# ashvardanian/StringZilla

Measured on AMD Instinct MI355X. Metric: DP cell-updates/s (GCUPS) on 1M-pair Levenshtein batch, higher is better.
Workload: dtype u32 bit-vectors (u64 results)

## Files before the change

### stringzilla_amd/csrc/hip/lev_myers.hip

```cpp
#include "myers_core.hpp"

#define SZS_PAIR_RULE_FN __host__ __device__ static inline
#include "pair_rule.h"
#define SZS_CORNER_CUT_FN __host__ __device__ static inline
#include "corner_cut.h"

#include <cstdlib>

namespace szs_hip {

#ifndef SZS_MYERS_PACK_QUERIES
#define SZS_MYERS_PACK_QUERIES 1
#endif
#ifndef SZS_MYERS_PAIR_RULES
#define SZS_MYERS_PAIR_RULES 1
#endif

#ifndef SZS_MYERS_CUT_CORNERS
#define SZS_MYERS_CUT_CORNERS 1
#endif

#ifndef SZS_MYERS_SHORT_TEXT_DWORDS
#define SZS_MYERS_SHORT_TEXT_DWORDS 2
#endif


__device__ __forceinline__ u32 bits_in_word(u32 from, u32 to, int w) {
    u32 const low = from > 32u * w ? from : 32u * w, high = to < 32u * w + 32u ? to : 32u * w + 32u;
    if (low >= high) return 0u;
    return (high - low == 32u ? ~0u : (1u << (high - low)) - 1u) << (low - 32u * w);
}

template <int words_, int text_dwords_, bool runes_, bool paired_ = false>
__device__ __forceinline__ void myers_workgroup(u32 *peq, u32 *keys, szs_string_ref_t const query,
                                                szs_string_ref_t const *__restrict__ candidates, u32 candidates_count,
                                                u32 candidate_block, u64 *__restrict__ results, u64 results_row_stride,
                                                int symmetric, szs_ref_guard_t const &guard, u32 alphabet = 0,
                                                u32 *claimed_rows = nullptr, u32 blocks_here = 1, szs_string_ref_t const second = {}) {
    static_assert(!paired_ || !runes_, "query pairs are a byte-kernel shape");
    constexpr int rows = runes_ ? rune_slots_k : byte_rows_k;
    using layout = peq_layout<words_, rows>;
    if (guard.enabled && (!ref_is_current(guard, 0, query) || (paired_ && !ref_is_current(guard, 0, second)))) {
        if (threadIdx.x == 0) *guard.stale = guard.sequence;
        return;
    }
    u32 const first_length = query.length, second_length = paired_ ? second.length : 0u;
    u32 const query_length = paired_ ? first_length + second_length : first_length;
    u32 const used_rows = paired_ ? query_length + 2u : query_length;
    u32 const pad = 32u * words_ - used_rows;
    u32 const second_row = pad + first_length + 2u;

    if constexpr (paired_) {
        u32 const s0_dword = (second_row - 2u) >> 5, s0_mask = 1u << ((second_row - 2u) & 31u);
        for (int i = threadIdx.x; i < layout::total_dwords; i += 256)
            peq[i] = (u32)(i / (rows * layout::chunk_words) * layout::chunk_words + i % layout::chunk_words) == s0_dword ? s0_mask : 0u;
    }
    else
        for (int i = threadIdx.x; i < layout::total_dwords; i += 256) peq[i] = 0;
    if constexpr (runes_) {
        if (alphabet) {
            for (u32 i = threadIdx.x; i <= alphabet; i += 256) keys[i] = 0;
            if (threadIdx.x == 0) *claimed_rows = 0;
        }
        else
            for (int i = threadIdx.x; i < rune_slots_k; i += 256) keys[i] = rune_slot_empty_k;
    }
    __syncthreads();
    if (runes_ && alphabet) {
        u32 const *pattern = reinterpret_cast<u32 const *>(query.address);
        for (u32 i = threadIdx.x; i < query_length; i += 256) {
            u32 const id = pattern[i];
            if (atomicCAS(&keys[id], 0u, ~0u) == 0u) keys[id] = atomicAdd(claimed_rows, 1u) + 1;
        }
        __syncthreads();
        for (u32 i = threadIdx.x; i < query_length; i += 256) {
            u32 const position = pad + i;
            atomicOr(&peq[layout::dword_index((int)keys[pattern[i]], (int)(position >> 5))], 1u << (position & 31));
        }
    }
    else if constexpr (runes_) {
        u32 const *pattern = reinterpret_cast<u32 const *>(query.address);
        for (u32 i = threadIdx.x; i < query_length; i += 256) {
            u32 const rune = pattern[i];
            u32 slot = rune_slot_hash(rune);
            for (;;) {
                u32 const previous = atomicCAS(&keys[slot], rune_slot_empty_k, rune);
                if (previous == rune_slot_empty_k || previous == rune) break;
                slot = (slot + 1) & (rune_slots_k - 1);
            }
            u32 const position = pad + i;
            atomicOr(&peq[layout::dword_index((int)slot, (int)(position >> 5))], 1u << (position & 31));
        }
    }
    else {
        u8 const *pattern = reinterpret_cast<u8 const *>(query.address);
        for (u32 i = threadIdx.x; i < first_length; i += 256) {
            u32 const position = pad + i;
            atomicOr(&peq[layout::dword_index(pattern[i], (int)(position >> 5))], 1u << (position & 31));
        }
        if constexpr (paired_) {
            u8 const *above = reinterpret_cast<u8 const *>(second.address);
            for (u32 i = threadIdx.x; i < second_length; i += 256) {
                u32 const position = second_row + i;
                atomicOr(&peq[layout::dword_index(above[i], (int)(position >> 5))], 1u << (position & 31));
            }
        }
    }
    __syncthreads();
    pattern_pair_t<words_> boundary;
    if constexpr (paired_) {
#pragma unroll
        for (int w = 0; w < words_; ++w) {
            boundary.separators[w] = bits_in_word(second_row - 2u, second_row, w);
            boundary.lower[w] = bits_in_word(second_row - 2u, second_row - 1u, w);
        }
    }

#pragma unroll 1
    for (u32 block_step = 0; block_step < blocks_here; ++block_step) {
    u32 const candidate_slot = (candidate_block - block_step) * SZS_CANDIDATES_PER_WORKGROUP + threadIdx.x;
    bool live = candidate_slot < candidates_count;
    szs_string_ref_t candidate = {0, 0, 0};
    if (live) candidate = candidates[candidate_slot];
    if (live && guard.enabled && !ref_is_current(guard, 1, candidate)) {
        *guard.stale = guard.sequence;
        live = false;
    }
    if ((symmetric & SZS_LAYOUT_SYMMETRIC) && candidate.index > query.index) live = false;
    u32 const text_length = live ? candidate.length : 0;
    u32 const longest_in_wave = wave_max_u32(text_length);
    u32 const shortest_in_wave = ~wave_max_u32(live ? ~text_length : 0u);

    u32 vp[words_], vn[words_];
#pragma unroll
    for (int w = 0; w < words_; ++w) {
        vp[w] = bits_in_word(pad, 32u * words_, w) & ~(paired_ ? boundary.separators[w] : 0u);
        vn[w] = 0;
    }

    auto take_words = [&](u32 symbol, auto first_word, auto last_word) {
        constexpr int first = decltype(first_word)::value, last = decltype(last_word)::value;
        u32 eq[words_];
        load_match_masks<words_, rows, first, last>(peq, !runes_ ? symbol : alphabet ? keys[symbol] : find_rune_slot(keys, symbol), eq);
        if constexpr (paired_) myers_column<words_, pattern_pair_t<words_>, true, true, first, last>(vp, vn, eq, boundary);
        else myers_column<words_, single_pattern_t, true, true, first, last>(vp, vn, eq);
    };
    constexpr std::integral_constant<int, 0> word_zero{};
    constexpr std::integral_constant<int, words_> word_end{};
    auto take = [&](u32 symbol) { take_words(symbol, word_zero, word_end); };

    u32 column = 0;
    if constexpr (runes_) {
        u32 const *const runes = reinterpret_cast<u32 const *>(candidate.address);
        auto quad_at = [&](u32 index) -> uint4 {
            return index < text_length ? *reinterpret_cast<uint4 const *>(runes + index) : make_uint4(0, 0, 0, 0);
        };
        if (4 <= shortest_in_wave && longest_in_wave) {
            uint4 ahead = quad_at(0);
            for (; column + 4 <= shortest_in_wave; column += 4) {
                uint4 const now = ahead;
                ahead = quad_at(column + 4);
                take(now.x), take(now.y), take(now.z), take(now.w);
            }
        }
#pragma unroll 1
        for (; column < longest_in_wave; ++column)
            if (column < text_length) take(runes[column]);
    }
    else {
        u64 const safe_address = text_length ? candidate.address : first_length || !paired_ ? query.address : second.address;
        text_stream_t text(safe_address, text_length);
        if (!text_length) text.valid_dwords = query_length ? 1 : 0;
        u32 raw_low = text.raw(0);
        u32 dword = 0;
        constexpr u32 columns_per_iteration = 4 * text_dwords_;
#ifndef SZS_MYERS_CLAMPED_READS
#define SZS_MYERS_CLAMPED_READS(TEXT_DWORDS) ((TEXT_DWORDS) == 1)
#endif
        constexpr bool clamped_reads = SZS_MYERS_CLAMPED_READS(text_dwords_);
        constexpr bool phases = SZS_MYERS_CUT_CORNERS && !runes_ && words_ >= (int)SZS_CORNER_CUT_WORDS_LEAST && text_dwords_ > 1;
        constexpr std::integral_constant<int, phases ? 1 : 0> word_one{};
        constexpr std::integral_constant<int, phases ? words_ - 1 : words_> word_top{};
        u32 head_until = 0, late_from = SZS_CORNER_CUT_NEVER;
        if constexpr (phases)
            szs_corner_cut(first_length, second_length, paired_, words_, (u32)__builtin_amdgcn_readfirstlane((int)shortest_in_wave),
                           (u32)__builtin_amdgcn_readfirstlane((int)longest_in_wave), &head_until, &late_from);
        if (columns_per_iteration <= shortest_in_wave && longest_in_wave && query_length) {
            u32 ahead[text_dwords_];
#pragma unroll
            for (int d = 0; d < text_dwords_; ++d) ahead[d] = clamped_reads ? text.raw_clamped(1 + d) : text.raw(1 + d);
            auto batch = [&](auto first_word, auto last_word) {
                u32 symbols[text_dwords_];
                symbols[0] = text.splice(raw_low, ahead[0]);
#pragma unroll
                for (int d = 1; d < text_dwords_; ++d) symbols[d] = text.splice(ahead[d - 1], ahead[d]);
                raw_low = ahead[text_dwords_ - 1];
#pragma unroll
                for (int d = 0; d < text_dwords_; ++d)
                    ahead[d] = clamped_reads ? text.raw_clamped(dword + text_dwords_ + 1 + d)
                                             : text.raw(dword + text_dwords_ + 1 + d);
#pragma unroll
                for (int step = 0; step < 4 * text_dwords_; ++step)
                    take_words((symbols[step / 4] >> (8 * (step % 4))) & 0xFFu, first_word, last_word);
                column += columns_per_iteration, dword += text_dwords_;
            };
            if constexpr (phases) {
                u32 const shortest = (u32)__builtin_amdgcn_readfirstlane((int)shortest_in_wave);
                u32 const head_end = head_until < shortest ? head_until : shortest;
                while (column + columns_per_iteration <= head_end) batch(word_zero, word_top);
            }
            while (column + columns_per_iteration <= shortest_in_wave && (!phases || column < late_from)) batch(word_zero, word_end);
            if constexpr (phases)
                while (column + columns_per_iteration <= shortest_in_wave) batch(word_one, word_end);
        }
#ifndef SZS_MYERS_MID_LOOP
#define SZS_MYERS_MID_LOOP 0
#endif
        if constexpr (SZS_MYERS_MID_LOOP && text_dwords_ > 1) {
            if (column + 4 <= shortest_in_wave && longest_in_wave && query_length) {
                u32 ahead_one = text.raw(dword + 1);
#pragma unroll 1
                for (; column + 4 <= shortest_in_wave; column += 4, ++dword) {
                    u32 const symbols = text.splice(raw_low, ahead_one);
                    raw_low = ahead_one;
                    ahead_one = text.raw(dword + 2);
#pragma unroll
                    for (int step = 0; step < 4; ++step) take((symbols >> (8 * step)) & 0xFFu);
                }
            }
        }
        if (column < longest_in_wave) {
            u32 next = text.raw(dword + 1);
#pragma unroll 1
            for (; column < longest_in_wave; column += 4, ++dword) {
                u32 const after = text.raw(dword + 2);
                u32 const symbols = text.splice(raw_low, next);
                raw_low = next, next = after;
                if (phases && column >= late_from) {
#pragma unroll
                    for (int step = 0; step < 4; ++step)
                        if (column + step < text_length) take_words((symbols >> (8 * step)) & 0xFFu, word_one, word_end);
                    continue;
                }
#pragma unroll
                for (int step = 0; step < 4; ++step)
                    if (column + step < text_length) take((symbols >> (8 * step)) & 0xFFu);
            }
        }
    }

    if (live && paired_) {
        u32 first = text_length, above = text_length;
#pragma unroll
        for (int w = 0; w < words_; ++w) {
            u32 const mine = bits_in_word(pad, pad + first_length, w), theirs = bits_in_word(second_row, 32u * words_, w);
            first += (u32)__builtin_popcount(vp[w] & mine) - (u32)__builtin_popcount(vn[w] & mine);
            above += (u32)__builtin_popcount(vp[w] & theirs) - (u32)__builtin_popcount(vn[w] & theirs);
        }
        bool const transposed = (symmetric & SZS_LAYOUT_TRANSPOSED) != 0;
        u64 const one = transposed ? candidate.index : query.index, two = transposed ? candidate.index : second.index;
        u64 const one_column = transposed ? query.index : candidate.index, two_column = transposed ? second.index : candidate.index;
        results[one * results_row_stride + one_column] = first;
        results[two * results_row_stride + two_column] = above;
    }
    else if (live) {
        u32 distance = text_length;
#pragma unroll
        for (int w = 0; w < words_; ++w) distance += (u32)__builtin_popcount(vp[w]) - (u32)__builtin_popcount(vn[w]);
        bool const transposed = (symmetric & SZS_LAYOUT_TRANSPOSED) != 0;
        u64 const row = transposed ? candidate.index : query.index, column = transposed ? query.index : candidate.index;
        results[row * results_row_stride + column] = distance;
        if ((symmetric & SZS_LAYOUT_SYMMETRIC) && candidate.index != query.index)
            results[column * results_row_stride + row] = distance;
    }
    }
}

#ifndef SZS_WORK_BLOCK_MAJOR
#define SZS_WORK_BLOCK_MAJOR 1
#endif
__device__ __forceinline__ void myers_work_item(u32 candidate_blocks, u32 &query_slot, u32 &candidate_block) {
#if SZS_WORK_BLOCK_MAJOR
    u32 const queries_count = gridDim.x / candidate_blocks;
    query_slot = blockIdx.x % queries_count;
    candidate_block = candidate_blocks - 1 - blockIdx.x / queries_count;
#else
    query_slot = blockIdx.x / candidate_blocks;
    candidate_block = candidate_blocks - 1 - blockIdx.x % candidate_blocks;
#endif
}

#ifndef SZS_MYERS_LONG_WAVES
#define SZS_MYERS_LONG_WAVES 2
#endif
template <int words_>
__global__ __launch_bounds__(256, SZS_MYERS_LONG_WAVES) void levenshtein_myers_long_kernel(szs_string_ref_t const *__restrict__ queries,
                                                                      szs_string_ref_t const *__restrict__ candidates,
                                                                      u32 candidates_count, u32 candidate_blocks,
                                                                      u64 *__restrict__ results, u64 results_row_stride,
                                                                      int symmetric, szs_ref_guard_t guard) {
    __shared__ __attribute__((aligned(16))) u32 peq[peq_layout<words_>::total_dwords];
    u32 query_slot, candidate_block;
    myers_work_item(candidate_blocks, query_slot, candidate_block);
    myers_workgroup<words_, 1, false>(peq, nullptr, queries[query_slot], candidates, candidates_count, candidate_block,
                                      results, results_row_stride, symmetric, guard);
}

__device__ __forceinline__ u64 fused_offset(void const *offsets, u32 wide, u64 index) {
    return wide ? static_cast<u64 const *>(offsets)[index] : (u64) static_cast<u32 const *>(offsets)[index];
}

__device__ __forceinline__ void fused_sort_side(szs_plan_side_t const &side, u32 is_query_side, u32 choose_rule, u32 sequence, u32 *ready,
                                                u32 second_ready, u32 withhold, szs_fused_side_report_t *report, u32 *histogram ,
                                                szs_string_ref_t *staged ) {
    constexpr u32 per_thread = SZS_FUSED_MOST_STRINGS / 256;
    u32 const tid = threadIdx.x, lane = tid & 63u, wave = tid >> 6, count = side.count;
    bool const one_pass = count <= SZS_FUSED_MOST_STRINGS;
    __shared__ u32 wave_bins[4], wave_longest[4], wave_status[4];
    __shared__ unsigned long long wave_symbols[4], wave_bands_systolic[4], wave_bands_chain[4], wave_squares[4];
    __shared__ u32 rule_words[256];

    u64 const began = wall_clock64();
    for (u32 bin = tid; bin < SZS_FUSED_BINS; bin += 256) histogram[bin] = 0;
    u64 from[per_thread], to[per_thread];
#pragma unroll
    for (u32 k = 0; k < per_thread; ++k) {
        u32 const i = tid + k * 256;
        from[k] = to[k] = 0;
        if (one_pass && i < count) from[k] = fused_offset(side.offsets, side.wide, i), to[k] = fused_offset(side.offsets, side.wide, (u64)i + 1);
    }
    __syncthreads();
    u32 bins[per_thread];
    u32 status = 0, longest = 0;
    u64 symbols = 0, bands_systolic = 0, bands_chain = 0, squares = 0;
    auto count_in = [&](u64 first, u64 last) -> u32 {
        if (last < first) return status |= SZS_PLAN_STATUS_DESCENDING, ~0u;
        if (last - first > 0xFFFFFFFFull) return status |= SZS_PLAN_STATUS_OVERFLOW, ~0u;
        u32 const length = (u32)(last - first);
        symbols += length, squares += (u64)length * length, longest = length > longest ? length : longest;
        bands_systolic += length ? (length + SZS_SYSTOLIC_BAND_ROWS - 1) / SZS_SYSTOLIC_BAND_ROWS : 1;
        bands_chain += length ? (length + SZS_MYERS_CHAIN_BAND_ROWS - 1) / SZS_MYERS_CHAIN_BAND_ROWS : 1;
        u32 const bin = length < SZS_FUSED_BINS - 1 ? length : SZS_FUSED_BINS - 1;
        atomicAdd(&histogram[bin], 1u);
        return bin;
    };
    if (one_pass) {
#pragma unroll
        for (u32 k = 0; k < per_thread; ++k) {
            bins[k] = ~0u;
            if (tid + k * 256 < count) bins[k] = count_in(from[k], to[k]);
        }
    }
    else {
#pragma unroll 1
        for (u32 first = 0; first < count; first += 1024) {
            u64 some_from[4], some_to[4];
#pragma unroll
            for (u32 k = 0; k < 4; ++k) {
                u32 const i = first + tid + k * 256;
                some_from[k] = some_to[k] = 0;
                if (i < count) some_from[k] = fused_offset(side.offsets, side.wide, i), some_to[k] = fused_offset(side.offsets, side.wide, (u64)i + 1);
            }
#pragma unroll
            for (u32 k = 0; k < 4; ++k)
                if (first + tid + k * 256 < count) (void)count_in(some_from[k], some_to[k]);
        }
// ... 70 lines not shown
                some_from[k] = some_to[k] = 0;
                if (i < count) some_from[k] = fused_offset(side.offsets, side.wide, i), some_to[k] = fused_offset(side.offsets, side.wide, (u64)i + 1);
            }
#pragma unroll
            for (u32 k = 0; k < 4; ++k) {
                u32 const i = first + tid + k * 256;
                if (i >= count) continue;
                u32 const length = status ? 0u : (u32)(some_to[k] - some_from[k]);
                szs_string_ref_t ref;
                ref.address = status ? side.base : side.base + some_from[k], ref.length = blank ? 0u : length, ref.index = i;
                u32 const position = status ? i : atomicAdd(&histogram[length < SZS_FUSED_BINS - 1 ? length : SZS_FUSED_BINS - 1], 1u);
                side.ascending[position] = ref, side.descending[count - 1 - position] = ref;
            }
        }
    }
    __syncthreads();
    if (tid == 0) report->ticks[3] = (u32)(wall_clock64() - began);
    u32 pairing = 0;
    if (choosing && wave == 0) {
        constexpr u32 strides = 256 / SZS_PAIR_RULE_CANDIDATES;
        u32 key = ~0u;
        if (lane < SZS_PAIR_RULE_CANDIDATES) {
            u32 total = 0;
#pragma unroll
            for (u32 k = 0; k < strides; ++k) total += rule_words[lane + k * SZS_PAIR_RULE_CANDIDATES];
            key = (total << 5) | lane;
        }
#pragma unroll
        for (int offset = 16; offset >= 1; offset >>= 1) {
            u32 const other = (u32)__shfl_xor((int)key, offset, 64);
            key = other < key ? other : key;
        }
        pairing = szs_pair_rule_candidate(key & 31u, pair_seconds);
    }
    if (tid == 0) {
        if (!withhold) {
            if (is_query_side)
                __hip_atomic_store(reinterpret_cast<u64 *>(ready), ((u64)pairing << 32) | sequence, __ATOMIC_RELEASE, __HIP_MEMORY_SCOPE_AGENT);
            else
                __hip_atomic_store(ready, sequence, __ATOMIC_RELEASE, __HIP_MEMORY_SCOPE_AGENT);
            if (second_ready) __hip_atomic_store(ready + 32, sequence, __ATOMIC_RELAXED, __HIP_MEMORY_SCOPE_AGENT);
        }
        report->ticks[4] = (u32)(wall_clock64() - began);
    }
#pragma unroll
    for (int offset = 32; offset >= 1; offset >>= 1) {
        symbols += ((u64)(u32)__shfl_xor((int)(u32)(symbols >> 32), offset, 64) << 32) | (u32)__shfl_xor((int)(u32)symbols, offset, 64);
        squares += ((u64)(u32)__shfl_xor((int)(u32)(squares >> 32), offset, 64) << 32) | (u32)__shfl_xor((int)(u32)squares, offset, 64);
        bands_systolic += ((u64)(u32)__shfl_xor((int)(u32)(bands_systolic >> 32), offset, 64) << 32) | (u32)__shfl_xor((int)(u32)bands_systolic, offset, 64);
        bands_chain += ((u64)(u32)__shfl_xor((int)(u32)(bands_chain >> 32), offset, 64) << 32) | (u32)__shfl_xor((int)(u32)bands_chain, offset, 64);
    }
    if (lane == 0) wave_symbols[wave] = symbols, wave_bands_systolic[wave] = bands_systolic, wave_bands_chain[wave] = bands_chain, wave_squares[wave] = squares;
    if (tid <= SZS_PLAN_RANK_SAMPLES) {
        u32 const rank = (u32)((u64)tid * (count ? count - 1 : 0) / SZS_PLAN_RANK_SAMPLES);
        report->rank_lengths[tid] = status || !count ? 0u : one_pass ? staged[rank].length : side.ascending[rank].length;
    }
    __syncthreads();
    if (tid == 0) {
        report->status = status, report->blank = blank, report->pairing = pairing;
        report->stats.count = count, report->stats.longest = longest;
        report->stats.symbols = wave_symbols[0] + wave_symbols[1] + wave_symbols[2] + wave_symbols[3];
        report->stats.bands_systolic = wave_bands_systolic[0] + wave_bands_systolic[1] + wave_bands_systolic[2] + wave_bands_systolic[3];
        report->stats.bands_chain = wave_bands_chain[0] + wave_bands_chain[1] + wave_bands_chain[2] + wave_bands_chain[3];
        report->squares = wave_squares[0] + wave_squares[1] + wave_squares[2] + wave_squares[3];
        report->sequence = sequence;
    }
}

__device__ __forceinline__ bool fused_prologue(szs_fused_plan_t const &plan, u32 *scratch, u32 &pairing) {
    __shared__ __attribute__((aligned(16))) szs_string_ref_t staged[SZS_FUSED_MOST_STRINGS];
    for (u32 s = 0; s < (plan.symmetric ? 1u : 2u); ++s)
        if (blockIdx.x == s % gridDim.x) {
            fused_sort_side(plan.side[s], s == 0, SZS_MYERS_PAIR_RULES && SZS_MYERS_PACK_QUERIES && s == 0 && !plan.symmetric && plan.blocks_per_group == 1,
                            plan.sequence, plan.ready + 32 * s, plan.symmetric, plan.withhold, plan.report + s, scratch, staged);
            __syncthreads();
        }
    __shared__ u32 unpublished[2], published_high[2];
    if (threadIdx.x < 2) {
        u32 polls = 0;
        u64 word;
        bool published;
        while (!(published = (u32)(word = __hip_atomic_load(reinterpret_cast<u64 const *>(plan.ready + 32 * threadIdx.x), __ATOMIC_RELAXED,
                                                             __HIP_MEMORY_SCOPE_AGENT)) == plan.sequence) &&
               ++polls < plan.poll_budget)
            __builtin_amdgcn_s_sleep(8);
        unpublished[threadIdx.x] = !published, published_high[threadIdx.x] = (u32)(word >> 32);
    }
    __syncthreads();
    pairing = (u32)__builtin_amdgcn_readfirstlane((int)published_high[0]);
    if (unpublished[0] | unpublished[1]) {
        if (threadIdx.x == 0) __hip_atomic_store(plan.gave_up, plan.sequence, __ATOMIC_RELAXED, __HIP_MEMORY_SCOPE_SYSTEM);
        return false;
    }
    return true;
}

#ifndef SZS_MYERS_SHORT_WAVES
#define SZS_MYERS_SHORT_WAVES 1
#endif
constexpr u32 szs_myers_pair_words_k = SZS_PAIR_WORDS_MOST;
template <bool runes_, bool merged_, bool fused_ = false>
__device__ __forceinline__ void myers_short_body(
    szs_string_ref_t const *__restrict__ queries, szs_string_ref_t const *__restrict__ candidates, u32 candidates_count,
    u32 candidate_blocks, u64 *__restrict__ results, u64 results_row_stride, int symmetric, szs_ref_guard_t guard, u32 alphabet,
    u32 blocks_per_group, szs_fused_plan_t const *fused = nullptr) {
    constexpr bool pairs = fused_ && !merged_ && SZS_MYERS_PACK_QUERIES;
    __shared__ __attribute__((aligned(16))) u32 peq[peq_layout<pairs ? szs_myers_pair_words_k : 8, runes_ ? rune_slots_k : byte_rows_k>::total_dwords];
    u32 pairing = 0;
    if constexpr (fused_) {
        static_assert(peq_layout<8, byte_rows_k>::total_dwords >= SZS_FUSED_BINS, "the sort's histogram borrows the masks' LDS");
        if (!fused_prologue(*fused, peq, pairing)) return;
    }
    __shared__ u32 slot_keys[runes_ ? rune_slots_k : 1];
    __shared__ u32 claimed_rows;
    extern __shared__ u32 rows_of_ids[];
    u32 *const keys = runes_ && alphabet ? rows_of_ids : slot_keys;
    u32 query_slot, candidate_group;
    myers_work_item(candidate_blocks, query_slot, candidate_group);
    u32 const all_blocks = (candidates_count + SZS_CANDIDATES_PER_WORKGROUP - 1) / SZS_CANDIDATES_PER_WORKGROUP;
    u32 const first_block = merged_ ? candidate_group * blocks_per_group : candidate_group;
    u32 const blocks_here = !merged_ ? 1u : all_blocks - first_block < blocks_per_group ? all_blocks - first_block : blocks_per_group;
    u32 const candidate_block = first_block + blocks_here - 1;
    szs_string_ref_t query = queries[query_slot];
    if constexpr (fused_) {
        query.address = ((u64)(u32)__builtin_amdgcn_readfirstlane((int)(u32)(query.address >> 32)) << 32) |
                        (u32)__builtin_amdgcn_readfirstlane((int)(u32)query.address);
        query.length = (u32)__builtin_amdgcn_readfirstlane((int)query.length);
        query.index = (u32)__builtin_amdgcn_readfirstlane((int)query.index);
    }
    szs_string_ref_t second = {0, 0, 0};
    bool has_second = false;
    if constexpr (pairs) {
        if (!fused->symmetric) {
            u32 const slots = szs_pair_slots(fused->side[0].count), seconds = szs_pair_seconds(fused->side[0].count);
            if (query_slot < seconds) {
                u32 rule = pairing;
                rule = rule <= seconds ? rule : 0u;
                second = queries[szs_pair_second_rank(rule, query_slot, slots, seconds)];
                second.address = ((u64)(u32)__builtin_amdgcn_readfirstlane((int)(u32)(second.address >> 32)) << 32) |
                                 (u32)__builtin_amdgcn_readfirstlane((int)(u32)second.address);
                second.length = (u32)__builtin_amdgcn_readfirstlane((int)second.length);
                second.index = (u32)__builtin_amdgcn_readfirstlane((int)second.index);
                has_second = true;
            }
        }
    }
    u32 const words = __builtin_amdgcn_readfirstlane(query.length ? (query.length + 31u) / 32u : 1u);
    u32 const second_words = second.length ? (second.length + 31u) / 32u : 1u;
    u32 const pair_words = szs_pair_words_shared(query.length, second.length);
    if constexpr (pairs) {
        if (has_second && szs_pair_shares(pair_words, words, second_words)) {
#define SZS_MYERS_PAIR_BODY(W)                                                                                         \
    case W:                                                                                                            \
        myers_workgroup<W, SZS_MYERS_SHORT_TEXT_DWORDS, false, true>(peq, keys, query, candidates, candidates_count,   \
                                                                     candidate_block, results, results_row_stride,    \
                                                                     symmetric, guard, 0u, nullptr, 1u, second);      \
        return;
            switch (pair_words) {
                SZS_MYERS_PAIR_BODY(1)
                SZS_MYERS_PAIR_BODY(2)
                SZS_MYERS_PAIR_BODY(3)
                SZS_MYERS_PAIR_BODY(4)
                SZS_MYERS_PAIR_BODY(5)
                SZS_MYERS_PAIR_BODY(6)
                SZS_MYERS_PAIR_BODY(7)
                SZS_MYERS_PAIR_BODY(8)
                SZS_MYERS_PAIR_BODY(9)
                SZS_MYERS_PAIR_BODY(10)
            }
#undef SZS_MYERS_PAIR_BODY
        }
    }
#define SZS_MYERS_BODY(W)                                                                                              \
    case W:                                                                                                            \
        myers_workgroup<W, SZS_MYERS_SHORT_TEXT_DWORDS, runes_>(peq, keys, query, candidates, candidates_count,       \
                                                                candidate_block, results, results_row_stride,         \
                                                                symmetric, guard, alphabet, &claimed_rows, blocks_here); \
        break;
    for (u32 turn = 0; turn < (has_second ? 2u : 1u); ++turn) {
        if (turn) {
            __syncthreads();
            query = second;
        }
        switch (turn ? second_words : words) {
            SZS_MYERS_BODY(1)
            SZS_MYERS_BODY(2)
            SZS_MYERS_BODY(3)
            SZS_MYERS_BODY(4)
            SZS_MYERS_BODY(5)
            SZS_MYERS_BODY(6)
            SZS_MYERS_BODY(7)
        default:
            myers_workgroup<8, SZS_MYERS_SHORT_TEXT_DWORDS, runes_>(peq, keys, query, candidates, candidates_count,
                                                                    candidate_block, results, results_row_stride, symmetric, guard,
                                                                    alphabet, &claimed_rows, blocks_here);
            break;
        }
    }
#undef SZS_MYERS_BODY
}

template <bool runes_>
__global__ __launch_bounds__(256, SZS_MYERS_SHORT_WAVES) void levenshtein_myers_short_kernel(
    szs_string_ref_t const *__restrict__ queries, szs_string_ref_t const *__restrict__ candidates, u32 candidates_count,
    u32 candidate_blocks, u64 *__restrict__ results, u64 results_row_stride, int symmetric, szs_ref_guard_t guard, u32 alphabet,
    u32 blocks_per_group) {
    myers_short_body<runes_, false>(queries, candidates, candidates_count, candidate_blocks, results, results_row_stride, symmetric, guard,
                                    alphabet, blocks_per_group);
}

#ifndef SZS_MYERS_FUSED_WAVES
#define SZS_MYERS_FUSED_WAVES 5
#endif
template <bool merged_>
__global__ __launch_bounds__(256, SZS_MYERS_FUSED_WAVES) void levenshtein_myers_short_fused_kernel(szs_fused_plan_t plan, u32 candidate_blocks,
                                                                                                   u64 *results, u64 results_row_stride,
                                                                                                   int layout) {
    szs_ref_guard_t const none = {};
    szs_plan_side_t const &texts = plan.symmetric ? plan.side[0] : plan.side[1];
    myers_short_body<false, merged_, true>(plan.side[0].descending, texts.ascending, texts.count, candidate_blocks, results, results_row_stride,
                                           layout, none, 0u, plan.blocks_per_group, &plan);
}

template <bool runes_>
__global__ __launch_bounds__(256, SZS_MYERS_SHORT_WAVES) void levenshtein_myers_short_merged_kernel(
    szs_string_ref_t const *__restrict__ queries, szs_string_ref_t const *__restrict__ candidates, u32 candidates_count,
    u32 candidate_blocks, u64 *__restrict__ results, u64 results_row_stride, int symmetric, szs_ref_guard_t guard, u32 alphabet,
    u32 blocks_per_group) {
    myers_short_body<runes_, true>(queries, candidates, candidates_count, candidate_blocks, results, results_row_stride, symmetric, guard,
                                   alphabet, blocks_per_group);
}

constexpr int banded_widest_k = 64;
constexpr size_t banded_header_bytes_k = 256;

template <int words_>
__device__ __forceinline__ i32 myers_strips(u32 *peq, szs_string_ref_t const query, u32 strips, text_stream_t const &text,
                                            u32 text_length, u32 shortest_in_wave, u32 longest_in_wave, u32 *parked_mine) {
    using layout = peq_layout<words_>;
    constexpr u32 strip_rows = 32u * words_;
    u32 const query_length = query.length;
    u32 const pad = strips * strip_rows - query_length;
    u8 const *const pattern = reinterpret_cast<u8 const *>(query.address);
    i32 delta_sum = 0;
    for (u32 strip = 0; strip < strips; ++strip) {
        bool const first_strip = strip == 0, last_strip = strip + 1 == strips;
        __syncthreads();
        for (int i = threadIdx.x; i < layout::total_dwords; i += 256) peq[i] = 0;
        __syncthreads();
        for (u32 bit = threadIdx.x; bit < strip_rows; bit += 256) {
            u32 const position = strip * strip_rows + bit;
            if (position >= pad) atomicOr(&peq[layout::dword_index(pattern[position - pad], (int)(bit >> 5))], 1u << (bit & 31));
        }
        __syncthreads();

        u32 vp[words_], vn[words_];
#pragma unroll
        for (int w = 0; w < words_; ++w) {
            u32 const first_bit = 32u * w;
            vp[w] = !first_strip || first_bit >= pad ? ~0u : (first_bit + 32u <= pad ? 0u : (~0u << (pad - first_bit)));
            vn[w] = 0;
        }

        u32 entering = 0, leaving = 0;
        auto take = [&](u32 symbol, u32 column) {
            u32 eq[words_];
            load_match_masks<words_, byte_rows_k>(peq, symbol, eq);
            u32 const slot = 2 * (column & 15u);
            u32 const hp_in = first_strip ? 1u : (entering >> slot) & 1u;
            u32 const hn_in = first_strip ? 0u : (entering >> (slot + 1)) & 1u;
            leaving |= myers_strip_column<words_>(vp, vn, eq, hp_in, hn_in) << slot;
        };

        u32 column = 0, dword = 0;
        u32 raw_low = text.raw(0);
        if (4 <= shortest_in_wave && longest_in_wave) {
            u32 ahead = text.raw_clamped(1);
            for (; column + 4 <= shortest_in_wave; column += 4, ++dword) {
                u32 const symbols = text.splice(raw_low, ahead);
                raw_low = ahead;
                ahead = text.raw_clamped(dword + 2);
                if ((dword & 3u) == 0) {
                    if (!first_strip) entering = parked_mine[(u64)(dword / 4) * 256];
                    leaving = 0;
                }
#pragma unroll 1
                for (int step = 0; step < 4; ++step) take((symbols >> (8 * step)) & 0xFFu, column + step);
                if ((dword & 3u) == 3 && !last_strip) parked_mine[(u64)(dword / 4) * 256] = leaving;
            }
        }
        if ((dword & 3u) != 0 && !last_strip) parked_mine[(u64)(dword / 4) * 256] = leaving;
        if (column < longest_in_wave) {
            u32 next = text.raw(dword + 1);
#pragma unroll 1
            for (; column < longest_in_wave; column += 4, ++dword) {
                u32 const after = text.raw(dword + 2);
                u32 const symbols = text.splice(raw_low, next);
                raw_low = next, next = after;
                if ((dword & 3u) == 0) {
                    if (!first_strip && column < text_length) entering = parked_mine[(u64)(dword / 4) * 256];
                    leaving = 0;
                }
#pragma unroll 1
                for (int step = 0; step < 4; ++step)
                    if (column + step < text_length) take((symbols >> (8 * step)) & 0xFFu, column + step);
                if (!last_strip && column < text_length && ((dword & 3u) == 3 || column + 4 >= text_length))
                    parked_mine[(u64)(dword / 4) * 256] = leaving;
            }
        }
#pragma unroll
        for (int w = 0; w < words_; ++w) delta_sum += (i32)__builtin_popcount(vp[w]) - (i32)__builtin_popcount(vn[w]);
    }
    return delta_sum;
}

__global__ __launch_bounds__(256, 2)  void levenshtein_myers_banded_kernel(szs_string_ref_t const *__restrict__ queries,
                                                                        u32 queries_count,
                                                                        szs_string_ref_t const *__restrict__ candidates,
                                                                        u32 candidates_count, u32 candidate_blocks,
                                                                        u64 *__restrict__ results, u64 results_row_stride,
                                                                        int symmetric, u32 *__restrict__ parked,
                                                                        u32 parked_dwords, u32 *__restrict__ work_counter) {
    __shared__ __attribute__((aligned(16))) u32 peq[peq_layout<banded_widest_k>::total_dwords];
    __shared__ u32 claimed_work;
    u32 *const parked_mine = parked + (u64)blockIdx.x * parked_dwords * 256 + threadIdx.x;

    u32 const work_items = queries_count * candidate_blocks;
    for (;;) {
        __syncthreads();
        if (threadIdx.x == 0) claimed_work = atomicAdd(work_counter, 1u);
        __syncthreads();
        u32 const work = claimed_work;
        if (work >= work_items) break;
        szs_string_ref_t const query = queries[work % queries_count];
        u32 const candidate_slot = (candidate_blocks - 1 - work / queries_count) * SZS_CANDIDATES_PER_WORKGROUP + threadIdx.x;
        bool live = candidate_slot < candidates_count;
        szs_string_ref_t candidate = {0, 0, 0};
        if (live) candidate = candidates[candidate_slot];
        if ((symmetric & SZS_LAYOUT_SYMMETRIC) && candidate.index > query.index) live = false;
        u32 const text_length = live ? candidate.length : 0;
        u32 const longest_in_wave = wave_max_u32(text_length);
        u32 const shortest_in_wave = ~wave_max_u32(live ? ~text_length : 0u);
        u64 const safe_address = text_length ? candidate.address : query.address;
        text_stream_t text(safe_address, text_length);
        if (!text_length) text.valid_dwords = query.length ? 1 : 0;

// ... 1012 lines not shown
```

### stringzilla_amd/csrc/hip/myers_core.hpp

```cpp
#pragma once
#include "device_common.hpp"

namespace szs_hip {

constexpr int byte_rows_k = 256;
constexpr int rune_slots_k = 512;
constexpr u32 rune_slot_empty_k = ~0u;

template <int words_, int rows_ = byte_rows_k>
struct peq_layout {
    static constexpr int chunk_words = words_ >= 3 ? 4 : words_;
    static constexpr int chunks = (words_ + chunk_words - 1) / chunk_words;
    static constexpr int total_dwords = chunks * rows_ * chunk_words;
    __device__ static constexpr int dword_index(int row, int w) {
        return ((w / chunk_words) * rows_ + row) * chunk_words + (w % chunk_words);
    }
};

__device__ __forceinline__ u32 rune_slot_hash(u32 rune) { return (rune * 2654435761u) >> 23; }
__device__ __forceinline__ u32 find_rune_slot(u32 const *keys, u32 rune) {
    u32 slot = rune_slot_hash(rune);
    for (;;) {
        u32 const key = keys[slot];
        if (key == rune || key == rune_slot_empty_k) return slot;
        slot = (slot + 1) & (rune_slots_k - 1);
    }
}

template <int words_, int rows_, int first_word_ = 0, int last_word_ = words_>
__device__ __forceinline__ void load_match_masks(u32 const *peq, u32 symbol, u32 (&eq)[words_]) {
    using layout = peq_layout<words_, rows_>;
    static_assert(0 <= first_word_ && first_word_ < last_word_ && last_word_ <= words_, "a word range inside the vector");
    if constexpr (layout::chunk_words == 4) {
        uint4 const *rows = reinterpret_cast<uint4 const *>(peq);
#pragma unroll
        for (int chunk = 0; chunk < layout::chunks; ++chunk) {
            if (chunk * 4 + 4 <= first_word_ || chunk * 4 >= last_word_) continue;
            uint4 const row = rows[chunk * rows_ + symbol];
            if (chunk * 4 < first_word_) asm volatile("" : : "v"(row.x));
            if (chunk * 4 + 0 < words_) eq[chunk * 4 + 0] = row.x;
            if (chunk * 4 + 1 < words_) eq[chunk * 4 + 1] = row.y;
            if (chunk * 4 + 2 < words_) eq[chunk * 4 + 2] = row.z;
            if (chunk * 4 + 3 < words_) eq[chunk * 4 + 3] = row.w;
        }
    }
    else if constexpr (layout::chunk_words == 2) {
        uint2 const row = reinterpret_cast<uint2 const *>(peq)[symbol];
        eq[0] = row.x, eq[1] = row.y;
    }
    else { eq[0] = peq[symbol]; }
}

__device__ __forceinline__ bool ref_is_current(szs_ref_guard_t const &guard, int side, szs_string_ref_t const &ref) {
    if (ref.index >= guard.side[side].count) return false;
    u64 from, to;
    if (guard.side[side].wide) {
        u64 const *offsets = static_cast<u64 const *>(guard.side[side].offsets);
        from = offsets[ref.index], to = offsets[(u64)ref.index + 1];
    }
    else {
        u32 const *offsets = static_cast<u32 const *>(guard.side[side].offsets);
        from = offsets[ref.index], to = offsets[(u64)ref.index + 1];
    }
    return to >= from && to - from == ref.length && guard.side[side].base + from == ref.address;
}

struct single_pattern_t {};

template <int words_>
struct pattern_pair_t {
    u32 separators[words_], lower[words_];
};

template <int table_>
__device__ __forceinline__ u32 bitop3(u32 a, u32 b, u32 c) {
    u32 r;
    asm("v_bitop3_b32 %0, %1, %2, %3 bitop3:%4" : "=v"(r) : "v"(a), "v"(b), "v"(c), "n"(table_));
    return r;
}

template <int words_, typename boundary_t = single_pattern_t, bool materialise_ = true, bool spelled_carries_ = true, int first_word_ = 0,
          int last_word_ = words_>
__device__ __forceinline__ void myers_column(u32 (&vp)[words_], u32 (&vn)[words_], u32 const (&eq)[words_],
                                             boundary_t const &boundary = {}) {
    constexpr bool paired = !std::is_same<boundary_t, single_pattern_t>::value;
    static_assert(spelled_carries_ || !paired, "a pair's HNs is not a function the compiler finds by itself");
    static_assert(0 <= first_word_ && first_word_ < last_word_ && last_word_ <= words_, "a word range inside the vector");
    u32 carry = 0, hp_below = 0;
#pragma unroll
    for (int w = first_word_; w < last_word_; ++w) {
        u32 xv, kept, hn_shifted;
        if constexpr (paired) {
            xv = bitop3<0xfe>(eq[w], vn[w], boundary.separators[w]);
            kept = bitop3<0x54>(eq[w], vp[w], boundary.lower[w]);
        }
        else
            xv = eq[w] | vn[w], kept = eq[w] | vp[w];
        u32 carry_out;
        u32 const sum = __builtin_addc(eq[w] & vp[w], vp[w], carry, &carry_out);
        carry = carry_out;
        if constexpr (paired) hn_shifted = bitop3<0x94>(sum, kept, eq[w]);
        else if constexpr (spelled_carries_) hn_shifted = bitop3<0x96>(sum, kept, eq[w]);
        else hn_shifted = sum ^ kept ^ eq[w];
        u32 const hp = bitop3<0xf1>(vn[w], sum, kept);
        u32 const hp_shifted = w == first_word_ ? ((hp << 1) | 1u) : __builtin_amdgcn_alignbit(hp, hp_below, 31);
        hp_below = hp;
        vp[w] = bitop3<0xf1>(hn_shifted, xv, hp_shifted);
        if constexpr (paired) vn[w] = bitop3<0x40>(hp_shifted, xv, boundary.separators[w]);
        else vn[w] = hp_shifted & xv;
        if constexpr (materialise_ && words_ > 1) asm("" : "+v"(vp[w]), "+v"(vn[w]));
    }
}

template <int words_>
__device__ __forceinline__ u32 myers_infix_column(u32 (&vp)[words_], u32 (&vn)[words_], u32 const (&eq)[words_]) {
    u32 carry = 0, hp_below = 0, hn_below = 0;
#pragma unroll
    for (int w = 0; w < words_; ++w) {
        u32 const xv = eq[w] | vn[w];
        u32 carry_out;
        u32 const sum = __builtin_addc(eq[w] & vp[w], vp[w], carry, &carry_out);
        carry = carry_out;
        u32 const d0 = (sum ^ vp[w]) | eq[w];
        u32 const hp = vn[w] | ~(d0 | vp[w]);
        u32 const hn = vp[w] & d0;
        u32 const hp_shifted = w == 0 ? (hp << 1) : __builtin_amdgcn_alignbit(hp, hp_below, 31);
        u32 const hn_shifted = w == 0 ? (hn << 1) : __builtin_amdgcn_alignbit(hn, hn_below, 31);
        hp_below = hp, hn_below = hn;
        vp[w] = hn_shifted | ~(xv | hp_shifted);
        vn[w] = hp_shifted & xv;
        if constexpr (words_ > 1) asm("" : "+v"(vp[w]), "+v"(vn[w]));
    }
    return (hp_below >> 31) | ((hn_below >> 31) << 1);
}

template <int words_>
__device__ __forceinline__ u32 myers_prefix_column(u32 (&vp)[words_], u32 (&vn)[words_], u32 const (&eq)[words_]) {
    u32 carry = 0, hp_below = 0, hn_below = 0;
#pragma unroll
    for (int w = 0; w < words_; ++w) {
        u32 const xv = eq[w] | vn[w];
        u32 carry_out;
        u32 const sum = __builtin_addc(eq[w] & vp[w], vp[w], carry, &carry_out);
        carry = carry_out;
        u32 const d0 = (sum ^ vp[w]) | eq[w];
        u32 const hp = vn[w] | ~(d0 | vp[w]);
        u32 const hn = vp[w] & d0;
        u32 const hp_shifted = w == 0 ? ((hp << 1) | 1u) : __builtin_amdgcn_alignbit(hp, hp_below, 31);
        u32 const hn_shifted = w == 0 ? (hn << 1) : __builtin_amdgcn_alignbit(hn, hn_below, 31);
        hp_below = hp, hn_below = hn;
        vp[w] = hn_shifted | ~(xv | hp_shifted);
        vn[w] = hp_shifted & xv;
        if constexpr (words_ > 1) asm("" : "+v"(vp[w]), "+v"(vn[w]));
    }
    return (hp_below >> 31) | ((hn_below >> 31) << 1);
}

template <int words_>
__device__ __forceinline__ u32 myers_prefix_column_traced(u32 (&vp)[words_], u32 (&vn)[words_], u32 const (&eq)[words_],
                                                          u32 (&diagonal_zero)[words_]) {
    u32 carry = 0, hp_below = 0, hn_below = 0;
#pragma unroll
    for (int w = 0; w < words_; ++w) {
        u32 const xv = eq[w] | vn[w];
        u32 carry_out;
        u32 const sum = __builtin_addc(eq[w] & vp[w], vp[w], carry, &carry_out);
        carry = carry_out;
        u32 const d0 = (sum ^ vp[w]) | eq[w];
        diagonal_zero[w] = d0 | vn[w];
        u32 const hp = vn[w] | ~(d0 | vp[w]);
        u32 const hn = vp[w] & d0;
        u32 const hp_shifted = w == 0 ? ((hp << 1) | 1u) : __builtin_amdgcn_alignbit(hp, hp_below, 31);
        u32 const hn_shifted = w == 0 ? (hn << 1) : __builtin_amdgcn_alignbit(hn, hn_below, 31);
        hp_below = hp, hn_below = hn;
        vp[w] = hn_shifted | ~(xv | hp_shifted);
        vn[w] = hp_shifted & xv;
        if constexpr (words_ > 1) asm("" : "+v"(vp[w]), "+v"(vn[w]));
    }
    return (hp_below >> 31) | ((hn_below >> 31) << 1);
}

template <int words_>
__device__ __forceinline__ u32 myers_strip_column(u32 (&vp)[words_], u32 (&vn)[words_], u32 const (&eq)[words_], u32 hp_in,
                                                  u32 hn_in) {
    u32 carry = 0, hp_below = 0, hn_below = 0;
#pragma unroll
    for (int w = 0; w < words_; ++w) {
        u32 const xv = eq[w] | vn[w];
        u32 const eq_in = w == 0 ? (eq[w] | hn_in) : eq[w];
        u32 carry_out;
        u32 const sum = __builtin_addc(eq_in & vp[w], vp[w], carry, &carry_out);
        carry = carry_out;
        u32 const d0 = (sum ^ vp[w]) | eq_in;
        u32 const hp = vn[w] | ~(d0 | vp[w]);
        u32 const hn = vp[w] & d0;
        u32 const hp_shifted = w == 0 ? ((hp << 1) | hp_in) : __builtin_amdgcn_alignbit(hp, hp_below, 31);
        u32 const hn_shifted = w == 0 ? ((hn << 1) | hn_in) : __builtin_amdgcn_alignbit(hn, hn_below, 31);
        hp_below = hp, hn_below = hn;
        vp[w] = hn_shifted | ~(xv | hp_shifted);
        vn[w] = hp_shifted & xv;
    }
    return (hp_below >> 31) | ((hn_below >> 31) << 1);
}

}
```

Measured before the change: 124,200.

## Prefetch next column's match masks and read text via global address space

```diff
diff --git a/stringzilla_amd/csrc/hip/lev_myers.hip b/stringzilla_amd/csrc/hip/lev_myers.hip
--- a/stringzilla_amd/csrc/hip/lev_myers.hip
+++ b/stringzilla_amd/csrc/hip/lev_myers.hip
@@ -20,10 +20,37 @@
 #define SZS_MYERS_CUT_CORNERS 1
 #endif
 
+#ifndef SZS_MYERS_SCALAR_MASKS_WORDS_LEAST
+#define SZS_MYERS_SCALAR_MASKS_WORDS_LEAST 1
+#endif
+
+#ifndef SZS_MYERS_GLOBAL_TEXT
+#define SZS_MYERS_GLOBAL_TEXT 1
+#endif
+#ifndef SZS_MYERS_COLUMN_AHEAD
+#define SZS_MYERS_COLUMN_AHEAD 1
+#endif
+#ifndef SZS_MYERS_COLUMN_AHEAD_MAY_CROSS
+#define SZS_MYERS_COLUMN_AHEAD_MAY_CROSS 0
+#endif
+
 #ifndef SZS_MYERS_SHORT_TEXT_DWORDS
 #define SZS_MYERS_SHORT_TEXT_DWORDS 2
 #endif
 
+
+struct global_text_stream_t : text_stream_t {
+    typedef u32 const __attribute__((address_space(1))) *global_dwords_t;
+    __device__ __forceinline__ global_text_stream_t(u64 address, u32 length) : text_stream_t(address, length) {}
+    __device__ __forceinline__ u32 raw(u32 dword_index) const {
+        return dword_index < valid_dwords ? ((global_dwords_t)aligned_base)[dword_index] : 0u;
+    }
+    __device__ __forceinline__ u32 raw_clamped(u32 dword_index) const {
+        return ((global_dwords_t)aligned_base)[dword_index < valid_dwords ? dword_index : valid_dwords - 1];
+    }
+};
+
+__host__ __device__ constexpr bool pair_masks_scalar(int words) { return SZS_MYERS_SCALAR_MASKS != 0 && words >= SZS_MYERS_SCALAR_MASKS_WORDS_LEAST; }
 
 __device__ __forceinline__ u32 bits_in_word(u32 from, u32 to, int w) {
     u32 const low = from > 32u * w ? from : 32u * w, high = to < 32u * w + 32u ? to : 32u * w + 32u;
@@ -31,7 +58,7 @@
     return (high - low == 32u ? ~0u : (1u << (high - low)) - 1u) << (low - 32u * w);
 }
 
-template <int words_, int text_dwords_, bool runes_, bool paired_ = false>
+template <int words_, int text_dwords_, bool runes_, bool paired_ = false, bool column_ahead_ = false>
 __device__ __forceinline__ void myers_workgroup(u32 *peq, u32 *keys, szs_string_ref_t const query,
                                                 szs_string_ref_t const *__restrict__ candidates, u32 candidates_count,
                                                 u32 candidate_block, u64 *__restrict__ results, u64 results_row_stride,
@@ -107,12 +134,17 @@
         }
     }
     __syncthreads();
-    pattern_pair_t<words_> boundary;
+    using boundary_of = pattern_pair_t<words_, pair_masks_scalar(words_)>;
+    boundary_of boundary;
     if constexpr (paired_) {
 #pragma unroll
         for (int w = 0; w < words_; ++w) {
             boundary.separators[w] = bits_in_word(second_row - 2u, second_row, w);
             boundary.lower[w] = bits_in_word(second_row - 2u, second_row - 1u, w);
+            if constexpr (boundary_of::scalar) {
+                boundary.separators[w] = (u32)__builtin_amdgcn_readfirstlane((int)boundary.separators[w]);
+                boundary.lower[w] = (u32)__builtin_amdgcn_readfirstlane((int)boundary.lower[w]);
+            }
         }
     }
 
@@ -138,12 +170,22 @@
         vn[w] = 0;
     }
 
+    constexpr bool builtin = builtin_bitop3_k && text_dwords_ > 1;
+    auto read_masks = [&](u32 symbol, u32 (&eq)[words_], auto first_word, auto last_word) {
+        constexpr int first = decltype(first_word)::value, last = decltype(last_word)::value;
+        load_match_masks<words_, rows, first, last, false>(peq, symbol, eq);
+    };
+    auto column_of = [&](u32 const (&eq)[words_], auto first_word, auto last_word, auto read_ahead) {
+        constexpr int first = decltype(first_word)::value, last = decltype(last_word)::value;
+        if constexpr (decltype(read_ahead)::value) use_skipped_mask<words_, first>(eq);
+        if constexpr (paired_) myers_column<words_, boundary_of, true, true, first, last, builtin>(vp, vn, eq, boundary);
+        else myers_column<words_, single_pattern_t, true, true, first, last, builtin>(vp, vn, eq);
+    };
     auto take_words = [&](u32 symbol, auto first_word, auto last_word) {
         constexpr int first = decltype(first_word)::value, last = decltype(last_word)::value;
         u32 eq[words_];
         load_match_masks<words_, rows, first, last>(peq, !runes_ ? symbol : alphabet ? keys[symbol] : find_rune_slot(keys, symbol), eq);
-        if constexpr (paired_) myers_column<words_, pattern_pair_t<words_>, true, true, first, last>(vp, vn, eq, boundary);
-        else myers_column<words_, single_pattern_t, true, true, first, last>(vp, vn, eq);
+        column_of(eq, first_word, last_word, std::false_type{});
     };
     constexpr std::integral_constant<int, 0> word_zero{};
     constexpr std::integral_constant<int, words_> word_end{};
@@ -169,7 +211,7 @@
     }
     else {
         u64 const safe_address = text_length ? candidate.address : first_length || !paired_ ? query.address : second.address;
-        text_stream_t text(safe_address, text_length);
+        std::conditional_t<SZS_MYERS_GLOBAL_TEXT != 0, global_text_stream_t, text_stream_t> text(safe_address, text_length);
         if (!text_length) text.valid_dwords = query_length ? 1 : 0;
         u32 raw_low = text.raw(0);
         u32 dword = 0;
@@ -189,9 +231,12 @@
             u32 ahead[text_dwords_];
 #pragma unroll
             for (int d = 0; d < text_dwords_; ++d) ahead[d] = clamped_reads ? text.raw_clamped(1 + d) : text.raw(1 + d);
+            constexpr bool column_ahead = SZS_MYERS_COLUMN_AHEAD && column_ahead_ && words_ >= 3 && text_dwords_ > 1;
+            static_assert(!column_ahead || columns_per_iteration % 2 == 0, "the set in flight at an iteration's end is the one its first column uses");
+            u32 masks_ahead[2][column_ahead ? words_ : 1], first_symbols = 0;
             auto batch = [&](auto first_word, auto last_word) {
                 u32 symbols[text_dwords_];
-                symbols[0] = text.splice(raw_low, ahead[0]);
+                symbols[0] = column_ahead ? first_symbols : text.splice(raw_low, ahead[0]);
 #pragma unroll
                 for (int d = 1; d < text_dwords_; ++d) symbols[d] = text.splice(ahead[d - 1], ahead[d]);
                 raw_low = ahead[text_dwords_ - 1];
@@ -199,19 +244,43 @@
                 for (int d = 0; d < text_dwords_; ++d)
                     ahead[d] = clamped_reads ? text.raw_clamped(dword + text_dwords_ + 1 + d)
                                              : text.raw(dword + text_dwords_ + 1 + d);
-#pragma unroll
-                for (int step = 0; step < 4 * text_dwords_; ++step)
-                    take_words((symbols[step / 4] >> (8 * (step % 4))) & 0xFFu, first_word, last_word);
+                if constexpr (column_ahead) {
+#pragma unroll
+                    for (int step = 0; step < 4 * text_dwords_; ++step) {
+                        if (step + 1 == 4 * text_dwords_) first_symbols = text.splice(raw_low, ahead[0]);
+                        u32 const next = step + 1 < 4 * text_dwords_ ? (symbols[(step + 1) / 4] >> (8 * ((step + 1) % 4))) & 0xFFu
+                                                                     : first_symbols & 0xFFu;
+                        read_masks(next, masks_ahead[(step + 1) % 2], first_word, last_word);
+                        __builtin_amdgcn_sched_barrier(SZS_MYERS_COLUMN_AHEAD_MAY_CROSS);
+                        column_of(masks_ahead[step % 2], first_word, last_word, std::true_type{});
+                    }
+                }
+                else {
+#pragma unroll
+                    for (int step = 0; step < 4 * text_dwords_; ++step)
+                        take_words((symbols[step / 4] >> (8 * (step % 4))) & 0xFFu, first_word, last_word);
+                }
                 column += columns_per_iteration, dword += text_dwords_;
+            };
+            auto loop = [&](auto first_word, auto last_word, auto more) {
+                if constexpr (column_ahead) {
+                    if (!more()) return;
+                    first_symbols = text.splice(raw_low, ahead[0]);
+                    read_masks(first_symbols & 0xFFu, masks_ahead[0], first_word, last_word);
+                    do batch(first_word, last_word);
+                    while (more());
+                }
+                else
+                    while (more()) batch(first_word, last_word);
             };
             if constexpr (phases) {
                 u32 const shortest = (u32)__builtin_amdgcn_readfirstlane((int)shortest_in_wave);
                 u32 const head_end = head_until < shortest ? head_until : shortest;
-                while (column + columns_per_iteration <= head_end) batch(word_zero, word_top);
-            }
-            while (column + columns_per_iteration <= shortest_in_wave && (!phases || column < late_from)) batch(word_zero, word_end);
+                loop(word_zero, word_top, [&] { return column + columns_per_iteration <= head_end; });
+            }
+            loop(word_zero, word_end, [&] { return column + columns_per_iteration <= shortest_in_wave && (!phases || column < late_from); });
             if constexpr (phases)
-                while (column + columns_per_iteration <= shortest_in_wave) batch(word_one, word_end);
+                loop(word_one, word_end, [&] { return column + columns_per_iteration <= shortest_in_wave; });
         }
 #ifndef SZS_MYERS_MID_LOOP
 #define SZS_MYERS_MID_LOOP 0
@@ -588,9 +657,9 @@
         if (has_second && szs_pair_shares(pair_words, words, second_words)) {
 #define SZS_MYERS_PAIR_BODY(W)                                                                                         \
     case W:                                                                                                            \
-        myers_workgroup<W, SZS_MYERS_SHORT_TEXT_DWORDS, false, true>(peq, keys, query, candidates, candidates_count,   \
-                                                                     candidate_block, results, results_row_stride,    \
-                                                                     symmetric, guard, 0u, nullptr, 1u, second);      \
+        myers_workgroup<W, SZS_MYERS_SHORT_TEXT_DWORDS, false, true, true>(peq, keys, query, candidates, candidates_count, \
+                                                                           candidate_block, results, results_row_stride, \
+                                                                           symmetric, guard, 0u, nullptr, 1u, second);   \
         return;
             switch (pair_words) {
                 SZS_MYERS_PAIR_BODY(1)
@@ -609,9 +678,9 @@
     }
 #define SZS_MYERS_BODY(W)                                                                                              \
     case W:                                                                                                            \
-        myers_workgroup<W, SZS_MYERS_SHORT_TEXT_DWORDS, runes_>(peq, keys, query, candidates, candidates_count,       \
-                                                                candidate_block, results, results_row_stride,         \
-                                                                symmetric, guard, alphabet, &claimed_rows, blocks_here); \
+        myers_workgroup<W, SZS_MYERS_SHORT_TEXT_DWORDS, runes_, false, !merged_>(                                     \
+            peq, keys, query, candidates, candidates_count, candidate_block, results, results_row_stride, symmetric, guard, alphabet,    \
+            &claimed_rows, blocks_here);                                                                                \
         break;
     for (u32 turn = 0; turn < (has_second ? 2u : 1u); ++turn) {
         if (turn) {
@@ -627,7 +696,7 @@
             SZS_MYERS_BODY(6)
             SZS_MYERS_BODY(7)
         default:
-            myers_workgroup<8, SZS_MYERS_SHORT_TEXT_DWORDS, runes_>(peq, keys, query, candidates, candidates_count,
+            myers_workgroup<8, SZS_MYERS_SHORT_TEXT_DWORDS, runes_, false, !merged_>(peq, keys, query, candidates, candidates_count,
                                                                     candidate_block, results, results_row_stride, symmetric, guard,
                                                                     alphabet, &claimed_rows, blocks_here);
             break;
diff --git a/stringzilla_amd/csrc/hip/myers_core.hpp b/stringzilla_amd/csrc/hip/myers_core.hpp
--- a/stringzilla_amd/csrc/hip/myers_core.hpp
+++ b/stringzilla_amd/csrc/hip/myers_core.hpp
@@ -27,7 +27,7 @@
     }
 }
 
-template <int words_, int rows_, int first_word_ = 0, int last_word_ = words_>
+template <int words_, int rows_, int first_word_ = 0, int last_word_ = words_, bool used_at_once_ = true>
 __device__ __forceinline__ void load_match_masks(u32 const *peq, u32 symbol, u32 (&eq)[words_]) {
     using layout = peq_layout<words_, rows_>;
     static_assert(0 <= first_word_ && first_word_ < last_word_ && last_word_ <= words_, "a word range inside the vector");
@@ -37,7 +37,7 @@
         for (int chunk = 0; chunk < layout::chunks; ++chunk) {
             if (chunk * 4 + 4 <= first_word_ || chunk * 4 >= last_word_) continue;
             uint4 const row = rows[chunk * rows_ + symbol];
-            if (chunk * 4 < first_word_) asm volatile("" : : "v"(row.x));
+            if (used_at_once_ && chunk * 4 < first_word_) asm volatile("" : : "v"(row.x));
             if (chunk * 4 + 0 < words_) eq[chunk * 4 + 0] = row.x;
             if (chunk * 4 + 1 < words_) eq[chunk * 4 + 1] = row.y;
             if (chunk * 4 + 2 < words_) eq[chunk * 4 + 2] = row.z;
@@ -49,6 +49,11 @@
         eq[0] = row.x, eq[1] = row.y;
     }
     else { eq[0] = peq[symbol]; }
+}
+
+template <int words_, int first_word_>
+__device__ __forceinline__ void use_skipped_mask(u32 const (&eq)[words_]) {
+    if constexpr (words_ >= 3 && first_word_ % 4 != 0) asm volatile("" : : "v"(eq[first_word_ / 4 * 4]));
 }
 
 __device__ __forceinline__ bool ref_is_current(szs_ref_guard_t const &guard, int side, szs_string_ref_t const &ref) {
@@ -67,20 +72,55 @@
 
 struct single_pattern_t {};
 
-template <int words_>
+#ifndef SZS_MYERS_SCALAR_MASKS
+#define SZS_MYERS_SCALAR_MASKS 0
+#endif
+#ifndef SZS_MYERS_BUILTIN_BITOP3
+#define SZS_MYERS_BUILTIN_BITOP3 0
+#endif
+#if !defined(__has_builtin)
+#define SZS_MYERS_HAS_BUILTIN_BITOP3 0
+#elif __has_builtin(__builtin_amdgcn_bitop3_b32)
+#define SZS_MYERS_HAS_BUILTIN_BITOP3 1
+#else
+#define SZS_MYERS_HAS_BUILTIN_BITOP3 0
+#endif
+constexpr bool builtin_bitop3_k = SZS_MYERS_BUILTIN_BITOP3 != 0 && SZS_MYERS_HAS_BUILTIN_BITOP3 != 0;
+
+template <int words_, bool scalar_ = SZS_MYERS_SCALAR_MASKS != 0>
 struct pattern_pair_t {
+    static constexpr bool scalar = scalar_;
     u32 separators[words_], lower[words_];
 };
 
-template <int table_>
+template <int table_, bool builtin_ = false>
 __device__ __forceinline__ u32 bitop3(u32 a, u32 b, u32 c) {
+#if SZS_MYERS_HAS_BUILTIN_BITOP3
+    if constexpr (builtin_) return __builtin_amdgcn_bitop3_b32(a, b, c, table_);
+#endif
     u32 r;
     asm("v_bitop3_b32 %0, %1, %2, %3 bitop3:%4" : "=v"(r) : "v"(a), "v"(b), "v"(c), "n"(table_));
     return r;
 }
 
+template <int table_, bool builtin_ = false>
+__device__ __forceinline__ u32 bitop3_scalar(u32 a, u32 b, u32 uniform_c) {
+#if SZS_MYERS_HAS_BUILTIN_BITOP3
+    if constexpr (builtin_) return __builtin_amdgcn_bitop3_b32(a, b, uniform_c, table_);
+#endif
+    u32 r;
+    asm("v_bitop3_b32 %0, %1, %2, %3 bitop3:%4" : "=v"(r) : "v"(a), "v"(b), "s"(uniform_c), "n"(table_));
+    return r;
+}
+
+template <int table_, typename boundary_t, bool builtin_ = false>
+__device__ __forceinline__ u32 bitop3_mask(u32 a, u32 b, u32 mask) {
+    if constexpr (boundary_t::scalar) return bitop3_scalar<table_, builtin_>(a, b, mask);
+    else return bitop3<table_, builtin_>(a, b, mask);
+}
+
 template <int words_, typename boundary_t = single_pattern_t, bool materialise_ = true, bool spelled_carries_ = true, int first_word_ = 0,
-          int last_word_ = words_>
+          int last_word_ = words_, bool builtin_ = false>
 __device__ __forceinline__ void myers_column(u32 (&vp)[words_], u32 (&vn)[words_], u32 const (&eq)[words_],
                                              boundary_t const &boundary = {}) {
     constexpr bool paired = !std::is_same<boundary_t, single_pattern_t>::value;
@@ -91,22 +131,22 @@
     for (int w = first_word_; w < last_word_; ++w) {
         u32 xv, kept, hn_shifted;
         if constexpr (paired) {
-            xv = bitop3<0xfe>(eq[w], vn[w], boundary.separators[w]);
-            kept = bitop3<0x54>(eq[w], vp[w], boundary.lower[w]);
+            xv = bitop3_mask<0xfe, boundary_t, builtin_>(eq[w], vn[w], boundary.separators[w]);
+            kept = bitop3_mask<0x54, boundary_t, builtin_>(eq[w], vp[w], boundary.lower[w]);
         }
         else
             xv = eq[w] | vn[w], kept = eq[w] | vp[w];
         u32 carry_out;
         u32 const sum = __builtin_addc(eq[w] & vp[w], vp[w], carry, &carry_out);
         carry = carry_out;
-        if constexpr (paired) hn_shifted = bitop3<0x94>(sum, kept, eq[w]);
-        else if constexpr (spelled_carries_) hn_shifted = bitop3<0x96>(sum, kept, eq[w]);
+        if constexpr (paired) hn_shifted = bitop3<0x94, builtin_>(sum, kept, eq[w]);
+        else if constexpr (spelled_carries_) hn_shifted = bitop3<0x96, builtin_>(sum, kept, eq[w]);
         else hn_shifted = sum ^ kept ^ eq[w];
-        u32 const hp = bitop3<0xf1>(vn[w], sum, kept);
+        u32 const hp = bitop3<0xf1, builtin_>(vn[w], sum, kept);
         u32 const hp_shifted = w == first_word_ ? ((hp << 1) | 1u) : __builtin_amdgcn_alignbit(hp, hp_below, 31);
         hp_below = hp;
-        vp[w] = bitop3<0xf1>(hn_shifted, xv, hp_shifted);
-        if constexpr (paired) vn[w] = bitop3<0x40>(hp_shifted, xv, boundary.separators[w]);
+        vp[w] = bitop3<0xf1, builtin_>(hn_shifted, xv, hp_shifted);
+        if constexpr (paired) vn[w] = bitop3_mask<0x40, boundary_t, builtin_>(hp_shifted, xv, boundary.separators[w]);
         else vn[w] = hp_shifted & xv;
         if constexpr (materialise_ && words_ > 1) asm("" : "+v"(vp[w]), "+v"(vn[w]));
     }
```

Measured after the change: 124,400 (median of 2 runs). About the same (+0.1%).
